# AnimatePortrait/AnimatePortrait

Hardware: AMD Instinct MI355X
Metric: generator frames/sec @256x256 bs=16 (higher is better)
Workload: dtype f32 (fp32 tensors; wide convs multiply fp32-class on the bf16 pipe: operands as bf16 head + tail, 3 products of 16-bit significands per multiply, ~2^-17 relative per product, fp32 accumulate); 1 GPU; Module2 generator resnet_9blocks_rcatland32_full_ifw fwd-only, ngf=64, bs=16/GPU, 256x256, fp32 (BASELINE configs[1]); global_batch=16, parallelism=dp1 (frame batches sharded, no collective), weights=random init N(0,0.02), seed 1234

## Files before the change

animateportrait_amd/csrc/conv_fwd.hip:

```cpp
#include "conv_plan.h"
#include "conv_direct.h"
#include "conv_tapgemm.h"
#include "conv_small.h"
#include "conv_head.h"
#include "conv_tsmall.h"

#include <cstdlib>
#include <cstring>

namespace apamd {

#ifdef APAMD_VARIANTS
const void* bf3_sb_kernel(size_t* lds_bytes);
#endif

static const void* direct_fn(int K, int cop) {
    if (K == 7 && cop == 1) return reinterpret_cast<const void*>(&conv_direct_f32<DirectCfg<7, 1>>);
    if (K == 7 && cop == 4) return reinterpret_cast<const void*>(&conv_direct_f32<DirectCfg<7, 4>>);
    return nullptr;
}
static size_t direct_lds_bytes(int K, int cop, int nbuf, int cin_pad) {
    if (cop == 1) return 4 * DirectCfg<7, 1>::lds_floats(nbuf, cin_pad);
    return 4 * DirectCfg<7, 4>::lds_floats(nbuf, cin_pad);
}

struct OutForm {
    const ap_out_view* view = nullptr;
    bool octet = false;
    bool bf16 = false;
};

struct FwdArgs {
    const float *packed, *bias;
    float *y, *stats;
    hipStream_t stream;
};

static int check_fwd_args(const ap_conv_desc* d, const Plan& pl, const OutForm& o, const FwdArgs& a) {
    if (o.bf16 && (!ob16_plan_ok(d, pl) || o.octet))
        return fail(AP_ERR_UNSUPPORTED, "conv2d_fwd_bf16out: only the plain-bf16 dense 3x3 stride-1 layers store bf16 (ap_conv2d_bf16out_ok)");
    if (!a.packed || !a.y) return fail(AP_ERR_INVALID, "null packed/y pointer");
    if (o.octet && !octet_plan_ok(d, pl))
        return fail(AP_ERR_UNSUPPORTED, "conv2d_fwd_octet: only single-launch split-bf16 layers of the run-time-tap / row kernel "
                                        "families with Cout %% 8 == 0 write the channel-octet layout (ap_conv2d_octet_ok)");
    if (o.view) {
        if (!pl.bf3 || pl.fused_phases || pl.launches.size() != 1)
            return fail(AP_ERR_UNSUPPORTED, "conv2d_fwd_view: only single-launch split-bf16 plans take an output window");
        if (o.view->OH < 1 || o.view->OW < 1 || o.view->OH > pl.Hout || o.view->OW > pl.Wout)
            return fail(AP_ERR_INVALID, "conv2d_fwd_view: window %dx%d outside the %dx%d output", o.view->OH, o.view->OW, pl.Hout, pl.Wout);
    }
    if (d->presplit && !pl.bf3) return fail(AP_ERR_INVALID, "desc.presplit set for a layer that does not take split sources");
    for (int s = 0; s < d->nsrc; ++s) {
        if (!d->src[s].data) return fail(AP_ERR_INVALID, "segment %d: null data", s);
        if ((d->src[s].mean == nullptr) != (d->src[s].rstd == nullptr))
            return fail(AP_ERR_INVALID, "segment %d: mean and rstd must be given together", s);
        if (d->src[s].act < 0 || d->src[s].act > 2) return fail(AP_ERR_INVALID, "segment %d: act %d", s, d->src[s].act);
    }
    return AP_OK;
}

static int launch_tsmall(const ap_conv_desc* d, const Plan& pl, const FwdArgs& a) {
    TSmallParams p;
    memset(&p, 0, sizeof(p));
    fill_seg(p.src, d->src[0], 0);
    p.N = d->N; p.C = pl.Cin; p.H = d->H; p.W = d->W; p.Cout = d->Cout;
    p.w = a.packed + pl.head_w_off; p.bias = a.bias; p.act = d->act; p.y = a.y;
    if (d->N > 65535 || (d->H + 7) / 8 > 65535) return fail(AP_ERR_UNSUPPORTED, "conv_tsmall: grid too large");
    const dim3 grid((d->W + 31) / 32, (d->H + 7) / 8, d->N);
    if (d->Cout == 1) hipLaunchKernelGGL((conv_tsmall_f32<1>), grid, dim3(256), 0, a.stream, p);
    else if (d->Cout == 2) hipLaunchKernelGGL((conv_tsmall_f32<2>), grid, dim3(256), 0, a.stream, p);
    else hipLaunchKernelGGL((conv_tsmall_f32<4>), grid, dim3(256), 0, a.stream, p);
    return check_launch("conv_tsmall_f32");
}

static int launch_head(const ap_conv_desc* d, const Plan& pl, const FwdArgs& a) {
    const int cus = num_cus();
    int rb = 3;
    long long best_cost = -1;
    for (int cand : {2, 3, 4, 5, 6, 10}) {
        const long long wgs = (long long)d->N * ((pl.Hout + cand - 1) / cand);
        const long long cost = ((wgs + cus - 1) / cus) * (cand + 3);
        if (best_cost < 0 || cost < best_cost) { rb = cand; best_cost = cost; }
    }
    HeadParams p;
    memset(&p, 0, sizeof(p));
    fill_seg(p.src, d->src[0], 0);
    p.N = d->N; p.C = pl.Cin; p.H = d->H; p.W = d->W; p.OH = pl.Hout; p.OW = pl.Wout;
    p.w = a.packed + pl.head_w_off; p.bias = a.bias; p.act = d->act; p.y = a.y;
    const dim3 hg(d->N, (pl.Hout + rb - 1) / rb);
    switch (rb) {
        case 2: hipLaunchKernelGGL(conv_head_fwd_kernel<2>, hg, dim3(1024), 0, a.stream, p); break;
        case 4: hipLaunchKernelGGL(conv_head_fwd_kernel<4>, hg, dim3(1024), 0, a.stream, p); break;
        case 5: hipLaunchKernelGGL(conv_head_fwd_kernel<5>, hg, dim3(1024), 0, a.stream, p); break;
        case 6: hipLaunchKernelGGL(conv_head_fwd_kernel<6>, hg, dim3(1024), 0, a.stream, p); break;
        case 10: hipLaunchKernelGGL(conv_head_fwd_kernel<10>, hg, dim3(1024), 0, a.stream, p); break;
        default: hipLaunchKernelGGL(conv_head_fwd_kernel<3>, hg, dim3(1024), 0, a.stream, p); break;
    }
    return check_launch("conv_head_fwd_kernel");
}

static int launch_small(const ap_conv_desc* d, const Plan& pl, const FwdArgs& a) {
    SmallKParams p;
    memset(&p, 0, sizeof(p));
    fill_seg(p.src, d->src[0], 0);
    p.N = d->N; p.H = d->H; p.W = d->W; p.Cin = pl.Cin; p.Cout = d->Cout; p.OH = pl.Hout; p.OW = pl.Wout;
    p.pad = d->pad; p.pad_mode = d->pad_mode;
    p.y = a.y; p.w = a.packed; p.bias = a.bias; p.act = d->act;
    p.stats = a.stats; p.stat_tiles = pl.stat_tiles;
    p.tiles_x = (pl.Wout + 31) / 32; p.tiles_y = (pl.Hout + 7) / 8;
    const dim3 grid((unsigned)((long long)d->N * p.tiles_y * p.tiles_x));
    if (d->stride == 1 && d->Cout == 8) hipLaunchKernelGGL((conv_small_f32<SmallCfg<1, 8>>), grid, dim3(256), 0, a.stream, p);
    else if (d->stride == 1) hipLaunchKernelGGL((conv_small_f32<SmallCfg<1, 16>>), grid, dim3(256), 0, a.stream, p);
    else if (d->Cout == 8) hipLaunchKernelGGL((conv_small_gather_f32<SmallCfg<2, 8>>), grid, dim3(256), 0, a.stream, p);
    else hipLaunchKernelGGL((conv_small_gather_f32<SmallCfg<2, 16>>), grid, dim3(256), 0, a.stream, p);
    return check_launch("conv_small_f32");
}

static bool tapgemm_serves(const ap_conv_desc* d, const Plan& pl, const FwdArgs& a) {
    return d->precision == AP_PRECISION_BF16X3 && d->Cout == 1 && d->KH == 7 && d->nsrc == 1 && d->src[0].C == TapGemmCfg::C &&
           d->pad_mode == AP_PAD_REFLECT && !a.stats && pl.cin_pad == TapGemmCfg::C;
}

static int launch_tapgemm(const ap_conv_desc* d, const Plan& pl, const FwdArgs& a) {
    const void* kfn = tapgemm_kernel();
    int rc = ensure_dyn_lds(kfn, 160 * 1024);
    if (rc) return rc;
    TapGemmParams p;
    memset(&p, 0, sizeof(p));
    fill_seg(p.seg, d->src[0], 0);
    p.N = d->N; p.H = d->H; p.W = d->W;
    p.y = a.y; p.wp = a.packed; p.bias = a.bias; p.act = d->act;
    p.tiles_x = (pl.Wout + TapGemmCfg::TW - 1) / TapGemmCfg::TW;
    const long long slots = 2LL * num_cus();
    long long best_cost = -1;
    for (int ty = 1; ty <= (pl.Hout + 7) / 8; ++ty) {
        const int th = (pl.Hout + ty - 1) / ty;
        const long long wgs = (long long)d->N * p.tiles_x * ((pl.Hout + th - 1) / th);
        const long long cost = ((wgs + slots - 1) / slots) * (th + 6);
        if (best_cost < 0 || cost < best_cost) { p.th = th; best_cost = cost; }
    }
    p.tiles_y = (pl.Hout + p.th - 1) / p.th;
    void* args[] = {&p};
    hipError_t e = hipLaunchKernel(kfn, dim3((unsigned)(d->N * p.tiles_y * p.tiles_x)), dim3(256), args, TapGemmCfg::lds_bytes(), a.stream);
    if (e != hipSuccess) return fail(AP_ERR_LAUNCH, "conv_tapgemm_bf16x3 launch: %s", hipGetErrorString(e));
    return AP_OK;
}

static int launch_direct(const ap_conv_desc* d, const Plan& pl, const FwdArgs& a) {
    if (tapgemm_serves(d, pl, a)) return launch_tapgemm(d, pl, a);
    const void* kfn = direct_fn(d->KH, pl.direct_cop);
    int rc = ensure_dyn_lds(kfn, 160 * 1024);
    if (rc) return rc;
    DirectKParams p;
    memset(&p, 0, sizeof(p));
    p.nseg = d->nsrc;
    for (int s = 0; s < d->nsrc; ++s) fill_seg(p.seg[s], d->src[s], pl.chunk_begin[s]);
    p.N = d->N; p.H = d->H; p.W = d->W; p.Cout = d->Cout; p.OH = pl.Hout; p.OW = pl.Wout;
    p.pad = d->pad; p.pad_mode = d->pad_mode;
    p.y = a.y; p.wp = a.packed; p.bias = a.bias; p.act = d->act;
    p.stats = a.stats; p.stat_tiles = pl.stat_tiles;
    p.nchunks = pl.nchunks; p.cin_pad = pl.cin_pad;
    p.tiles_x = (pl.Wout + 63) / 64; p.tiles_y = (pl.Hout + 15) / 16;
    const size_t lds = direct_lds_bytes(d->KH, pl.direct_cop, p.nchunks > 1 ? 2 : 1, p.cin_pad);
    void* args[] = {&p};
    hipError_t e = hipLaunchKernel(kfn, dim3((unsigned)(d->N * p.tiles_y * p.tiles_x)), dim3(256), args, lds, a.stream);
    if (e != hipSuccess) return fail(AP_ERR_LAUNCH, "conv_direct_f32 launch: %s", hipGetErrorString(e));
    return AP_OK;
}

static ConvKParams conv_params(const ap_conv_desc* d, const Plan& pl, const Launch& L, const FwdArgs& a, bool with_norm) {
    ConvKParams p;
    memset(&p, 0, sizeof(p));
    p.nseg = d->nsrc;
    for (int s = 0; s < d->nsrc; ++s) fill_seg(p.seg[s], d->src[s], pl.chunk_begin[s], with_norm);
    p.N = d->N; p.H = d->H; p.W = d->W; p.Cout = d->Cout;
    p.OH = L.OH; p.OW = L.OW; p.dy0 = L.dy0; p.dx0 = L.dx0;
    p.pad_mode = d->pad_mode; p.y = a.y;
    p.o_nstride = (long long)d->Cout * pl.Hout * pl.Wout; p.o_cstride = (long long)pl.Hout * pl.Wout; p.o_rstride = pl.Wout;
    p.osy = L.osy; p.osx = L.osx; p.oy_off = L.oy_off; p.ox_off = L.ox_off;
    p.wp = a.packed + L.wp_off; p.bias = a.bias; p.act = d->act;
    p.stats = a.stats; p.stat_tiles = pl.stat_tiles; p.stat_tile_off = L.stat_tile_off;
    p.ntaps = (int)L.taps.size(); p.nchunks = pl.nchunks;
    p.tiles_x = L.tiles_x; p.tiles_y = L.tiles_y; p.co_tiles = pl.co_tiles;
    p.cin_pad = pl.cin_pad;
// ... 214 lines not shown
```

animateportrait_amd/networks.py:

```python
import functools

import torch
import torch.nn as nn
from torch.optim import lr_scheduler

from . import ops
from .autograd import (conv_forward, materialize_forward, warp_forward, batch_split_forward,
                       generator_apply, discriminator_apply)
from .ops import (Feat, ConvSpec, ACT_NONE, ACT_RELU, ACT_LRELU, ACT_TANH, PAD_ZERO, PAD_REFLECT,
                  W_OIHW, W_IOHW)

GENERATOR_NAMES = ('resnet_9blocks_rcatland32_full_ifw', 'resnet_style2_9blocks')
_REFERENCE_ONLY_G = (
    'resnet_9blocks', 'resnet_9blocks_rcatland', 'resnet_9blocks_rcatland3',
    'resnet_9blocks_rcatland32', 'resnet_10blocks_rcatland32', 'resnet_9blocks_rcatland4',
    'resnet_9blocks_rcatland32_fw', 'resnet_9blocks_rcatland32_fw2', 'resnet_9blocks_rcatland32_ifw',
    'resnet_9blocks_rcatland32_ifw_single2', 'resnet_9blocks_rcatland32_full_ifw_colorcoded',
    'resnet_9blocks_rcatland32_full_ifw2', 'resnet_9blocks_rcatland32_full_ifw_single',
    'resnet_9blocks_rcatland32_full_ifw_single2', 'resnet_9blocks_rcatland32_full_ifw_single3', 'regressor',
    'combiner', 'resnet_9blocks_rcatland2', 'resnet_6blocks', 'unet_128', 'unet_256')


class ConvLayer(nn.Module):

    def __init__(self, cin_segments, cout, k, stride=1, pad=0, pad_mode=PAD_ZERO, transposed=False,
                 output_padding=0):
        super().__init__()
        cin = sum(cin_segments)
        shape = (cin, cout, k, k) if transposed else (cout, cin, k, k)
        self.weight = nn.Parameter(torch.empty(shape, dtype=torch.float32))
        self.bias = nn.Parameter(torch.zeros(cout, dtype=torch.float32))
        self.spec = ConvSpec(cin_segments, cout, k, stride, pad, pad_mode, transposed, output_padding,
                             W_IOHW if transposed else W_OIHW)
        self._slots = {}
        self._rows_spec = None
        self._s2d_spec = None

    def _packed(self, slot_id, spec, view):
        slot = ops.packed_slot(spec, self.weight, view, self._slots.get(slot_id))
        self._slots[slot_id] = slot
        return slot.buf

    def packed_dgrad(self, seg, spec, view):
        return self._packed(('dgrad', seg), spec, ops.WeightView(view))

    def packed(self):
        return self._packed('fwd', self.spec, ops.WeightView(self.weight.detach()))

    def run(self, srcs, norm_act=None, act=ACT_NONE, out_octet=False, out_bf16=False):
        if not isinstance(srcs, (list, tuple)):
            srcs = [srcs]
        spec, packed = self.spec, None
        if norm_act is None and ops.conv_d0_ok(spec, srcs, act):
            return ops.conv_d0(srcs[0], self.weight, self.bias.detach(), act)
        if ops.stem_rows_eligible(spec) and not srcs[0].is_split_only:
            spec, packed = self.rows_spec(), self.packed_rows()
            srcs = [ops.presplit_rows(srcs[0], self.spec.k, self.spec.pad, self.spec.pad_mode)]
        elif (srcs[0].s2d is not None or not srcs[0].is_split_only) and ops.s2d_eligible(spec, *srcs[0].data.shape[2:]):
            spec, packed = self.s2d_spec(), self.packed_s2d()
            if srcs[0].s2d is None:
                srcs[0].s2d = ops.presplit_s2d(srcs[0])
            srcs = [srcs[0].s2d]
        if packed is None:
            packed = self.packed()
        if norm_act is None:
            return ops.conv2d(spec, srcs, packed, self.bias.detach(), act=act, out_octet=out_octet)
        return ops.conv2d(spec, srcs, packed, None, want_stats=True, out_act=norm_act, out_octet=out_octet,
                          out_bf16=out_bf16 and spec is self.spec)

    def stages_split(self, shape):
        n, _, h, w = shape
        if ops.stem_rows_eligible(self.spec) or ops.s2d_eligible(self.spec, h, w):
            return False
        return ops.takes_split(self.spec, n, h, w)

    def s2d_spec(self):
        if self._s2d_spec is None:
            self._s2d_spec = ops.s2d_spec(self.spec)
        return self._s2d_spec

    def packed_s2d(self):
        return self._packed('s2d', self.s2d_spec(), ops.WeightView(self.weight.detach(), s2d_c=self.spec.cin_segments[0]))

    def rows_spec(self):
        if self._rows_spec is None:
            self._rows_spec = ops.stem_rows_spec(self.spec)
        return self._rows_spec

    def packed_rows(self):
        return self._packed('rows', self.rows_spec(), ops.WeightView(self.weight.detach(), rows_c=self.spec.cin_segments[0]))


def _seq(**children):
    return nn.ModuleDict({k.lstrip('_'): v for k, v in children.items()})


class ResnetBlock(nn.Module):

    def __init__(self, dim):
        super().__init__()
        self.conv_block = _seq(_1=ConvLayer([dim], dim, 3, 1, 1, PAD_REFLECT),
                               _5=ConvLayer([dim], dim, 3, 1, 1, PAD_REFLECT))

    def run(self, x, tape=None, consumer=None):
        c1, c5 = self.conv_block['1'], self.conv_block['5']
        dim = c1.spec.cout
        keep = consumer is not None and not consumer.stages_split(x.data.shape)
        y = conv_forward(tape, c1, x, norm_act=ACT_RELU, raw16=True, out_octet=tape is None and ops.trunk_octet_ok(dim))
        y = conv_forward(tape, c5, y, norm_act=ACT_NONE, raw16=True,
                         out_octet=tape is None and ops.trunk_octet_ok(dim, residual=x, keep_fp32=keep))
        return materialize_forward(tape, y, residual=x, consumer=consumer)


class ResnetBlock2(nn.Module):

    def __init__(self, segs, dim_out):
        super().__init__()
        self.conv_block = _seq(_1=ConvLayer(segs, dim_out, 3, 1, 1, PAD_REFLECT),
                               _5=ConvLayer([dim_out], dim_out, 3, 1, 1, PAD_REFLECT))
        self.shortcut = _seq(_0=ConvLayer(segs, dim_out, 3, 1, 1, PAD_ZERO))

    def run(self, srcs, tape=None, consumer=None):
        c1, c5, sc = self.conv_block['1'], self.conv_block['5'], self.shortcut['0']
        y = conv_forward(tape, c1, srcs, norm_act=ACT_RELU, raw16=True, out_octet=tape is None and ops.trunk_octet_ok(c1.spec.cout))
        y = conv_forward(tape, c5, y, norm_act=ACT_NONE, raw16=True)
        s = conv_forward(tape, sc, srcs, norm_act=ACT_NONE)
        return materialize_forward(tape, y, residual=s, consumer=consumer)


class ResnetConditionTriGenerator32_full_ifw(nn.Module):

    def __init__(self, input_nc, output_nc, ngf=64, norm='instance', use_dropout=False, n_blocks=9,
                 padding_type='reflect', div=3, disp=1):
        super().__init__()
        if norm != 'instance':
            raise NotImplementedError('normalization layer [%s] is not available on the HIP path' % norm)
        if use_dropout:
            raise NotImplementedError('dropout is not available on the HIP path (the model sets no_dropout)')
        if padding_type != 'reflect':
            raise NotImplementedError('padding [%s] is not implemented' % padding_type)
        assert n_blocks >= 0
        self.n_blocks, self.div, self.disp = n_blocks, div, disp
        self.input_nc, self.output_nc, self.ngf = input_nc, output_nc, ngf
        h = ngf // 2
        con_dim = 16
        dim = ngf * 4
        self.model_tri_merge = ConvLayer([ngf * 4, ngf * 4, ngf * 4], dim, 3, 1, 1)
        self.model_tri00 = _seq(_1=ConvLayer([input_nc], h, 7, 1, 3, PAD_REFLECT))
        self.model_tri01 = _seq(_0=ConvLayer([ngf], ngf * 2, 3, 2, 1))
        self.model_tri02 = _seq(_0=ConvLayer([ngf * 2], ngf * 4, 3, 2, 1))
        self.model_tri10 = _seq(_1=ConvLayer([input_nc], ngf, 7, 1, 3, PAD_REFLECT))
        self.model_tri11 = _seq(_0=ConvLayer([ngf], ngf, 3, 2, 1))
        self.model_tri12 = _seq(_0=ConvLayer([ngf * 2], ngf * 4, 3, 2, 1))
        self.model_tri20 = _seq(_1=ConvLayer([input_nc], ngf, 7, 1, 3, PAD_REFLECT))
        self.model_tri21 = _seq(_0=ConvLayer([ngf], ngf * 2, 3, 2, 1))
        self.model_tri22 = _seq(_0=ConvLayer([ngf * 2], ngf * 2, 3, 2, 1))
        blocks = {}
        for i in range(n_blocks):
            if (i + disp) % div == 0:
                blocks[str(i)] = ResnetBlock2([dim, con_dim, con_dim], dim)
            else:
                blocks[str(i)] = ResnetBlock(dim)
        self.model2 = nn.ModuleDict(blocks)
        self.model3 = _seq(_0=ConvLayer([ngf * 4], ngf * 2, 3, 2, 1, transposed=True, output_padding=1),
                           _3=ConvLayer([ngf * 2], ngf, 3, 2, 1, transposed=True, output_padding=1),
                           _7=ConvLayer([ngf], output_nc, 7, 1, 3, PAD_REFLECT))
        self.model_landmark_trans = _seq(_0=ConvLayer([1], 8, 3, 1, 1), _3=ConvLayer([8], con_dim, 3, 2, 1),
                                         _6=ConvLayer([con_dim], con_dim, 3, 2, 1))
        self.land1_cache_key = None
        self._land1_cache = None

    def is_block2(self, i):
        return (i + self.disp) % self.div == 0

    def double_feature_warping(self, x, motion, flow, ifmask, level, tape=None, consumer=None):
        return warp_forward(tape, x, motion, flow, ifmask, level, consumer=consumer)

    def forward(self, input, land1, land2, motion, flow, ifmask):
        if torch.is_grad_enabled() and (input.requires_grad or any(p.requires_grad for p in self.parameters())):
            return generator_apply(self, input, land1, land2, motion, flow, ifmask)
        return self.forward_inference(input, land1, land2, motion, flow, ifmask)

    def forward_inference(self, input, land1, land2, motion, flow, ifmask):
        return self._run(None, False, input, land1, land2, motion, flow, ifmask).data

    def _run(self, tape, input_needs_grad, input, land1, land2, motion, flow, ifmask):
        b = input.shape[0]
        inp = Feat(input.contiguous())
        if tape is not None and input_needs_grad:
            tape.track(inp)
        self._last_input_feat = inp if tape is not None else None
        motion, flow, ifmask = motion.contiguous(), flow.contiguous(), ifmask.contiguous()
        cf, dfw = conv_forward, self.double_feature_warping
        oct = tape is None

        def branch1():
            x = cf(tape, self.model_tri00['1'], inp, norm_act=ACT_RELU, out_octet=oct)
            x = dfw(x, motion, flow, ifmask, 0, tape, self.model_tri01['0'])
            x = cf(tape, self.model_tri01['0'], x, norm_act=ACT_RELU)
            return cf(tape, self.model_tri02['0'], x, norm_act=ACT_RELU)

        def branch2():
            x = cf(tape, self.model_tri10['1'], inp, norm_act=ACT_RELU)
            x = cf(tape, self.model_tri11['0'], x, norm_act=ACT_RELU, out_octet=oct)
            x = dfw(x, motion, flow, ifmask, 1, tape, self.model_tri12['0'])
            return cf(tape, self.model_tri12['0'], x, norm_act=ACT_RELU)

        def branch3():
            x = cf(tape, self.model_tri20['1'], inp, norm_act=ACT_RELU)
            x = cf(tape, self.model_tri21['0'], x, norm_act=ACT_RELU)
            x = cf(tape, self.model_tri22['0'], x, norm_act=ACT_RELU, out_octet=oct)
            return dfw(x, motion, flow, ifmask, 2, tape, self.model_tri_merge)

        def landmarks():
            lt = self.model_landmark_trans
            key = self.land1_cache_key
            if tape is None and key is not None:
                full = (key, tuple(land1.shape), tuple(ops.weight_key(lt[k].weight) for k in ('0', '3', '6')))
                if self._land1_cache is None or self._land1_cache[0] != full:
                    l = cf(None, lt['0'], Feat(land1.contiguous()), norm_act=ACT_RELU)
                    l = cf(None, lt['3'], l, norm_act=ACT_RELU)
                    l = cf(None, lt['6'], l, norm_act=ACT_NONE)
                    l.mean
                    self._land1_cache = (full, l)
                la = self._land1_cache[1]
                lb = cf(None, lt['0'], Feat(land2.contiguous()), norm_act=ACT_RELU)
                lb = cf(None, lt['3'], lb, norm_act=ACT_RELU)
                lb = cf(None, lt['6'], lb, norm_act=ACT_NONE)
                return la, lb
            lands = Feat(torch.cat([land1, land2], 0).contiguous())
            l = cf(tape, lt['0'], lands, norm_act=ACT_RELU)
            l = cf(tape, lt['3'], l, norm_act=ACT_RELU)
            l = cf(tape, lt['6'], l, norm_act=ACT_NONE)
            return batch_split_forward(tape, l, b)

        x1, x2, x3 = branch1(), branch2(), branch3()
        l1, l2 = landmarks()
        x = cf(tape, self.model_tri_merge, [x1, x2, x3])
        for i in range(self.n_blocks):
            blk = self.model2[str(i)]
            nxt = self.model3['0'] if i == self.n_blocks - 1 else None
            x = blk.run([x, l1, l2], tape, consumer=nxt) if self.is_block2(i) else blk.run(x, tape, consumer=nxt)
        x = cf(tape, self.model3['0'], x, norm_act=ACT_RELU)
        x = cf(tape, self.model3['3'], x, norm_act=ACT_RELU)
        return cf(tape, self.model3['7'], x, act=ACT_TANH)


class ResnetStyle2Generator(nn.Module):

    def __init__(self, input_nc, output_nc, ngf=64, norm='instance', use_dropout=False, n_blocks=6,
                 padding_type='reflect', extra_channel=3, model0_res=0):
        super().__init__()
        if norm != 'instance':
            raise NotImplementedError('normalization layer [%s] is not available on the HIP path' % norm)
        if use_dropout:
            raise NotImplementedError('dropout is not available on the HIP path')
        if padding_type != 'reflect':
            raise NotImplementedError('padding [%s] is not implemented' % padding_type)
        if model0_res != 0:
            raise NotImplementedError('model0_res != 0 is not used by any shipped configuration')
        assert n_blocks >= 0
        self.n_blocks = n_blocks
        dim = ngf * 4
        self.model0 = _seq(_1=ConvLayer([input_nc], ngf, 7, 1, 3, PAD_REFLECT),
                           _4=ConvLayer([ngf], ngf * 2, 3, 2, 1), _7=ConvLayer([ngf * 2], dim, 3, 2, 1))
        layers = {'0': ConvLayer([dim, extra_channel], dim, 3, 1, 1)}
        for i in range(n_blocks):
            layers[str(3 + i)] = ResnetBlock(dim)
        j = 3 + n_blocks
        layers[str(j)] = ConvLayer([dim], dim // 2, 3, 2, 1, transposed=True, output_padding=1)
        layers[str(j + 3)] = ConvLayer([dim // 2], dim // 4, 3, 2, 1, transposed=True, output_padding=1)
        layers[str(j + 7)] = ConvLayer([ngf], output_nc, 7, 1, 3, PAD_REFLECT)
        self.model = nn.ModuleDict(layers)

    def forward(self, input1, input2):
        with torch.no_grad():
            cf = conv_forward
            x = cf(None, self.model0['1'], Feat(input1.contiguous()), norm_act=ACT_RELU)
            x = cf(None, self.model0['4'], x, norm_act=ACT_RELU)
            x = cf(None, self.model0['7'], x, norm_act=ACT_RELU)
            x = cf(None, self.model['0'], [x, Feat(input2.contiguous())], norm_act=ACT_RELU)
            x = materialize_forward(None, x)
            j = 3 + self.n_blocks
            for i in range(self.n_blocks):
                x = self.model[str(3 + i)].run(x, None, consumer=self.model[str(j)] if i == self.n_blocks - 1 else None)
            x = cf(None, self.model[str(j)], x, norm_act=ACT_RELU)
            x = cf(None, self.model[str(j + 3)], x, norm_act=ACT_RELU)
            return cf(None, self.model[str(j + 7)], x, act=ACT_TANH).data


class P2CConv(ConvLayer):

    def __init__(self, cin, cout, k, stride=1, pad=0, pad_mode=PAD_ZERO, bias=False):
        super().__init__([cin], cout, k, stride, pad, pad_mode)
        self.spec.precision = ops.PRECISION_FP32
        nn.init.normal_(self.weight.data, 0.0, 0.02)
        if not bias:
            self.register_parameter('bias', None)

    def run(self, src, norm_act=None, act=ACT_NONE):
        if norm_act is None:
            return ops.conv2d(self.spec, [src], self.packed(), None if self.bias is None else self.bias.detach(), act=act)
        return ops.conv2d(self.spec, [src], self.packed(), None, want_stats=True, out_act=norm_act)


def _in_relu(t):
    return Feat(t[0], t[1], t[2], ACT_RELU)


class P2CConvBlock(nn.Module):

    def __init__(self, dim_in, dim_out):
        super().__init__()
        self.dim_in, self.dim_out = dim_in, dim_out
        self.ConvBlock1 = _seq(_3=P2CConv(dim_in, dim_out // 2, 3, 1, 1, PAD_REFLECT))
# ... 365 lines not shown
```

animateportrait_amd/ops.py:

```python
import collections
import ctypes
import os

import torch

from . import _capi as C
from ._capi import ACT_NONE, ACT_RELU, ACT_LRELU, ACT_TANH, PAD_ZERO, PAD_REFLECT, W_OIHW, W_IOHW

EPS = 1e-5

WEIGHTS_EPOCH = 0


def weight_key(w):
    owner = getattr(w, '_flat_owner', None)
    return (w._version, w.data_ptr(), WEIGHTS_EPOCH, owner.epoch if owner is not None else 0)

PRECISION_FP32, PRECISION_BF16X3, PRECISION_BF16 = 0, 1, 2
PRECISION_BY_NAME = {'fp32': PRECISION_FP32, 'bf16x3': PRECISION_BF16X3, 'bf16': PRECISION_BF16}
DEFAULT_PRECISION = PRECISION_BY_NAME.get(os.environ.get('APAMD_PRECISION', 'bf16x3'), PRECISION_BF16X3)


_LAST_STREAM = {}
_STREAM_FENCE = os.environ.get('APAMD_NO_STREAM_FENCE', '0') != '1'
# ... 442 lines not shown
    f.pending = None
    if want_xs and residual is None:
        f.xs = xs
        f.xs_heads_only = bool(flags & 1)
    return y, xs


def trunk_octet_ok(c, residual=None, keep_fp32=False):
    if (DEFAULT_PRECISION != PRECISION_BF16X3 or not RESIDUAL_AS_SPLIT or not OCTET_TRUNK or keep_fp32 or
            not wants_split(c) or c % 8):
        return False
    return residual is None or (residual.is_split_only and residual.xs is not None and not residual.xs_heads_only and residual.oct is None)


OCTET_TRUNK = os.environ.get('APAMD_NO_OCTET_TRUNK', '0') != '1'


def wants_split(c):
    return DEFAULT_PRECISION != PRECISION_FP32 and c >= 48 and c % 16 == 0


def takes_split(spec, n, h, w):
    if spec.precision == PRECISION_FP32:
        return False
    d = spec.desc(n, h, w)
    return bool(C.check(C.lib().ap_conv2d_wants_presplit(ctypes.byref(d)), 'wants_presplit'))


def conv2d(spec, srcs, packed, bias=None, act=ACT_NONE, want_stats=False, out_act=ACT_NONE, out_octet=False, out_bf16=False):
    x0 = srcs[0].data
    n, _, h, w = x0.shape
    for f, c in zip(srcs, spec.cin_segments):
        if not f.is_split_only:
            _require_device(f.data, 'conv input', allow_bf16=True)
        if f.data.shape[1] != c or f.data.shape[0] != n or f.data.shape[2:] != x0.shape[2:]:
            raise ValueError('conv2d: source of shape %s does not match segment C=%d' % (tuple(f.data.shape), c))
    d = spec.desc(n, h, w, None, act)
    lib = C.lib()
    if spec.precision != PRECISION_FP32 and C.check(lib.ap_conv2d_wants_presplit(ctypes.byref(d)), 'wants_presplit'):
        if spec.precision == PRECISION_BF16X3 and DEFAULT_PRECISION == PRECISION_BF16:
            raise RuntimeError('a split-bf16 (bf16x3) layer cannot run while the package mode is plain bf16: split copies '
                               'are then written without their tail planes')
        spec.presplit_desc(n, h, w, srcs, d=d)
    else:
        if any(f.is_split_only for f in srcs):
            raise RuntimeError('conv2d: a source exists only as its split-bf16 copy but this layer reads fp32')
        if any(f.data.dtype != torch.float32 for f in srcs):
            raise RuntimeError('conv2d: a source holds bf16 values but this layer reads fp32')
        spec.fill_sources(d, srcs)
    ho, wo = ctypes.c_int32(), ctypes.c_int32()
    C.check(lib.ap_conv2d_out_size(ctypes.byref(d), ctypes.byref(ho), ctypes.byref(wo)), 'conv2d_out_size')
    out_octet = bool(out_octet) and d.presplit == 1 and lib.ap_conv2d_octet_ok(ctypes.byref(d)) == 1
    out_bf16 = bool(out_bf16) and not out_octet and d.presplit == 1 and lib.ap_conv2d_bf16out_ok(ctypes.byref(d)) == 1
    if out_octet:
        y = torch.empty((n, spec.cout // 8, ho.value * wo.value, 8), dtype=torch.float32, device=x0.device)
    else:
        y = torch.empty((n, spec.cout, ho.value, wo.value), dtype=torch.bfloat16 if out_bf16 else torch.float32, device=x0.device)
    partial = None
    if want_stats:
        tiles = C.check(lib.ap_conv2d_stat_tiles(ctypes.byref(d)), 'conv2d_stat_tiles')
        partial = torch.empty((n * spec.cout, tiles, 2), dtype=torch.float32, device=x0.device)
    if PROFILER is not None:
        buf = ctypes.create_string_buffer(96)
        C.check(lib.ap_conv2d_kernel_name(ctypes.byref(d), buf, 96), 'conv2d_kernel_name')
        e0, e1 = torch.cuda.Event(enable_timing=True), torch.cuda.Event(enable_timing=True)
        e0.record()
    fwd = lib.ap_conv2d_fwd_octet if out_octet else (lib.ap_conv2d_fwd_bf16out if out_bf16 else lib.ap_conv2d_fwd)
    C.check(fwd(ctypes.byref(d), _ptr(packed), _ptr(bias), _ptr(y), _ptr(partial), _stream()), 'conv2d_fwd')
    if PROFILER is not None:
        e1.record()
        px = h * w if spec.transposed else ho.value * wo.value
        macs = getattr(spec, 'alg_macs', None) or sum(spec.cin_segments) * spec.k ** 2
        PROFILER.records.append((buf.value.decode(), 2.0 * n * px * spec.cout * macs, e0, e1))
    if out_octet:
        res = Feat(_stand_in((n, spec.cout, ho.value, wo.value), x0.device),
                   act=out_act if want_stats else ACT_NONE, pending=(partial, tiles) if want_stats else None)
        res.oct = y
        return res
    if not want_stats:
        return Feat(y)
    return Feat(y, act=out_act, pending=(partial, tiles))


RESIDUAL_AS_SPLIT = True
K7_WGRAD = os.environ.get('APAMD_NO_K7_WGRAD', '0') != '1'
D0_MFMA = K7_WGRAD and os.environ.get('APAMD_NO_D0_MFMA', '0') != '1'


def _conv2d_view(spec, srcs, packed, out, view):
    x0 = srcs[0].data
    n, _, h, w = x0.shape
    d = spec.presplit_desc(n, h, w, srcs)
    fn = C.lib().ap_conv2d_fwd_view_bf16out if out.dtype == torch.bfloat16 else C.lib().ap_conv2d_fwd_view
    C.check(fn(ctypes.byref(d), ctypes.byref(view), _ptr(packed), None, _ptr(out), _stream()), 'conv2d_fwd_view')


def dgrad_strip_eligible(spec, g):
    if (spec.precision == PRECISION_FP32 or spec.k != 3 or spec.stride != 1 or spec.pad != 2 or spec.transposed or
            len(spec.cin_segments) != 1 or g.virtual):
        return False
    n, c, h, w = g.shape
    if (w + 2) % 32 != 2 or w < 32 or h < 4 or c % 8:
        return False
    d = spec.desc(n, h, w, None, ACT_NONE)
    return bool(C.check(C.lib().ap_conv2d_wants_presplit(ctypes.byref(d)), 'wants_presplit'))


def conv2d_dgrad_strip(spec, g, packed, packed_t, strip=None, out_bf16=False):
    n, c, h, w = g.data.shape
    hp, wp = h + 2, w + 2
    out_bf16 = bool(out_bf16) and C.lib().ap_conv2d_bf16out_ok(ctypes.byref(spec.presplit_desc(n, h, w))) == 1
    out = torch.empty((n, spec.cout, hp, wp), dtype=torch.bfloat16 if out_bf16 else torch.float32, device=g.data.device)
    if strip is None and g.is_split_only:
        raise RuntimeError('conv2d_dgrad_strip: the gradient exists only as its split copy and no column strip was prepared '
                           '(ap_instnorm_bwd_split writes it when the backward plan asks for one)')
    t = strip if strip is not None else Feat(g.data[:, :, :, w - 2:].transpose(2, 3).contiguous())
    _conv2d_view(spec, [t], packed_t, out, C.ApOutView(spec.cout * hp * wp, hp * wp, 1, wp, w - 2, 0, 4, hp))
    _conv2d_view(spec, [g], packed, out, C.ApOutView(spec.cout * hp * wp, hp * wp, wp, 1, 0, 0, hp, w))
    return out


def materialize(f, residual=None, emit_xs=None, keep_fp32=True):
    if not f.virtual:
        raise ValueError('materialize: feature is already plain')
    n, c, h, w = f.data.shape
    if emit_xs is None:
        emit_xs = wants_split(c)
    if c % 8 == 0:
        split_only = (bool(emit_xs) and not keep_fp32 and RESIDUAL_AS_SPLIT and
                      DEFAULT_PRECISION == PRECISION_BF16X3)
        if residual is not None and residual.is_split_only and not split_only and residual.xs_heads_only:
            raise RuntimeError('materialize: the residual exists only as a head-only split copy')
        y, xs = _norm_apply_split(f, residual, want_y=not split_only, want_xs=bool(emit_xs))
        out = Feat.split_only((n, c, h, w), xs) if split_only else Feat(y)
        out.xs = xs
        out.xs_heads_only = xs is not None and DEFAULT_PRECISION == PRECISION_BF16
        return out
    x = f.data
    out = torch.empty_like(x)
    res = rm = rr = None
    if residual is not None:
        if residual.act != ACT_NONE and residual.virtual:
            raise ValueError('materialize: a normalised residual cannot carry an activation')
        res, rm, rr = residual.data, residual.mean, residual.rstd
        if res.shape != x.shape:
            raise ValueError('materialize: residual shape mismatch')
    C.check(C.lib().ap_instnorm_apply(_ptr(x), _ptr(f.mean), _ptr(f.rstd), f.act, _ptr(res), _ptr(rm), _ptr(rr),
                                      _ptr(out), n * c, h * w, _stream()), 'instnorm_apply')
    return Feat(out)


def warp_concat(f, motion, flow, ifmask, level, emit_xs=False, keep_fp32=True, s2d=False):
    x = f.data
    n, c, h, w = x.shape
    if f.oct is not None:
        x = f.oct
    for t, name in ((x, 'x'), (motion, 'motion'), (flow, 'flow'), (ifmask, 'ifmask')):
        _require_device(t, name)
    s = motion.shape[1]
    if motion.shape != (n, s, s, 2) or flow.shape != (n, 2, s, s) or ifmask.shape != (n, 1, s, s):
        raise ValueError('warp_concat: motion/flow/ifmask shapes %s %s %s' % (motion.shape, flow.shape, ifmask.shape))
    if h != s >> level or w != s >> level:
        raise ValueError('warp_concat: level %d expects %d px features, got %dx%d' % (level, s >> level, h, w))
    emit_xs = bool(emit_xs) and c % 8 == 0
    s2d = bool(s2d) and emit_xs and h % 2 == 0 and w % 2 == 0
    out = xs = None
# ... 502 lines not shown
```

include/animateportrait_amd.h:

```cpp
#ifndef ANIMATEPORTRAIT_AMD_H
#define ANIMATEPORTRAIT_AMD_H

#include <stdint.h>

#ifdef __cplusplus
extern "C" {
#endif

typedef void* ap_stream_t;

enum { AP_OK = 0, AP_ERR_INVALID = -1, AP_ERR_UNSUPPORTED = -2, AP_ERR_LAUNCH = -3 };
enum { AP_ACT_NONE = 0, AP_ACT_RELU = 1, AP_ACT_LRELU = 2 , AP_ACT_TANH = 3 };
enum { AP_PAD_ZERO = 0, AP_PAD_REFLECT = 1 };
enum { AP_W_OIHW = 0 , AP_W_IOHW = 1  };
enum { AP_PRECISION_FP32 = 0, AP_PRECISION_BF16X3 = 1, AP_PRECISION_BF16 = 2 };

typedef struct ap_src {
    const float* data;
    const float* mean;
    const float* rstd;
    int32_t C;
    int32_t act;
} ap_src;

typedef struct ap_conv_desc {
    int32_t N, H, W;
    int32_t Cout;
    int32_t KH, KW;
    int32_t stride;
    int32_t pad;
    int32_t pad_mode;
    int32_t transposed;
    int32_t output_padding;
    int32_t w_layout;
    int32_t w_flip;
    int32_t act;
    int32_t nsrc;
    int32_t precision;
    int32_t presplit;
    int32_t s2d_k;
    ap_src src[3];
} ap_conv_desc;

#define AP_ABI_VERSION 16
int32_t ap_abi_version(void);
const char* ap_version(void);
const char* ap_last_error(void);

int ap_conv2d_out_size(const ap_conv_desc* d, int32_t* Hout, int32_t* Wout);
int64_t ap_conv2d_packed_floats(const ap_conv_desc* d);
int32_t ap_conv2d_stat_tiles(const ap_conv_desc* d);
int ap_conv2d_pack_weights(const ap_conv_desc* d, const float* weight, float* packed, ap_stream_t stream);

typedef struct ap_weight_view {
    const float* w;
    int64_t s_co, s_ci, s_ky, s_kx;
    int32_t s2d_c, rows_c, ksrc, reserved;
} ap_weight_view;
int32_t ap_conv2d_pack_entry_bytes(void);
int32_t ap_conv2d_pack_entries(const ap_conv_desc* d, const ap_weight_view* v, float* packed, void* entries, int32_t max_entries);
int ap_conv2d_pack_run(const void* entries_dev, int32_t count, ap_stream_t stream);
int ap_conv2d_fwd(const ap_conv_desc* d, const float* packed, const float* bias, float* y,
                  float* stat_partials, ap_stream_t stream);
typedef struct ap_out_view {
    int64_t nstride, cstride;
    int32_t rstride, xstride, y_off, x_off, OH, OW;
} ap_out_view;
int ap_conv2d_fwd_view(const ap_conv_desc* d, const ap_out_view* view, const float* packed, const float* bias, float* y,
                       ap_stream_t stream);
int32_t ap_conv2d_octet_ok(const ap_conv_desc* d);
int ap_conv2d_fwd_octet(const ap_conv_desc* d, const float* packed, const float* bias, float* y, float* stat_partials,
                        ap_stream_t stream);
int32_t ap_conv2d_bf16out_ok(const ap_conv_desc* d);
int ap_conv2d_fwd_bf16out(const ap_conv_desc* d, const float* packed, const float* bias, void* y_bf16, float* stat_partials,
                          ap_stream_t stream);
int ap_conv2d_fwd_view_bf16out(const ap_conv_desc* d, const ap_out_view* view, const float* packed, const float* bias, void* y_bf16,
                               ap_stream_t stream);

int32_t ap_conv2d_wants_presplit(const ap_conv_desc* d);
int64_t ap_split_prepass_bytes(int32_t N, int32_t C, int32_t H, int32_t W);
int ap_split_prepass(const ap_src* src, int32_t N, int32_t H, int32_t W, void* out, ap_stream_t stream);
int ap_split_prepass_rows(const ap_src* src, int32_t N, int32_t H, int32_t W, int32_t K, int32_t pad, int32_t pad_mode,
                          void* out, ap_stream_t stream);
int ap_split_prepass_s2d(const ap_src* src, int32_t N, int32_t H, int32_t W, void* out, ap_stream_t stream);
int ap_norm_apply_split(const ap_src* src, const float* stat_partials, int32_t tiles, float eps, float* mean_out,
                        float* rstd_out, const ap_src* residual, int32_t N, int32_t H, int32_t W, float* y, void* xs,
                        ap_stream_t stream);
int ap_norm_apply_split_ex(const ap_src* src, const float* stat_partials, int32_t tiles, float eps, float* mean_out,
                           float* rstd_out, const ap_src* residual, int32_t N, int32_t H, int32_t W, float* y, void* xs,
                           int32_t flags, ap_stream_t stream);

int ap_conv2d_kernel_name(const ap_conv_desc* d, char* buf, int32_t buflen);

int ap_instnorm_finalize(const float* stat_partials, const float* y, int32_t NC, int32_t tiles, int32_t count,
                         float eps, float* mean, float* rstd, ap_stream_t stream);
int ap_instnorm_finalize_octet(const float* stat_partials, const float* y, int32_t N, int32_t C, int32_t tiles, int32_t count,
                               float eps, float* mean, float* rstd, ap_stream_t stream);
int ap_instnorm_apply(const float* x, const float* mean, const float* rstd, int32_t act,
                      const float* res, const float* res_mean, const float* res_rstd,
                      float* out, int32_t NC, int32_t HW, ap_stream_t stream);

int ap_warp_concat_fwd(const float* x, const float* x_mean, const float* x_rstd, int32_t x_act,
                       const float* motion, const float* flow, const float* ifmask,
                       float* out, int32_t N, int32_t C, int32_t H, int32_t W, int32_t S,
                       float flow_scale, ap_stream_t stream);
int ap_motion_grid(const float* pts, const float* val, const int32_t* tri, int32_t N, int32_t P, int32_t T, int32_t S,
// ... 129 lines not shown
```

Baseline: 2426 frames/s.

## Fuse landmark encoder layers 0 and 1 by recomputing layer-0 output on the fly

Replaces the stored 1->8 stride-1 landmark conv (with its full 8-channel activation write and reread) by a statistics-only pass that produces instance-norm sums, followed by a fused kernel. The fused kernel recomputes the 1->8 conv per tile in shared memory, applies norm and ReLU, and runs the 8->16 stride-2 conv with its stats epilogue. This removes the largest intermediate memory traffic of the landmark branch. In exchange it computes layer 0 twice and adds a halo of redundant work per tile.

```diff
diff --git a/animateportrait_amd/csrc/conv_fwd.hip b/animateportrait_amd/csrc/conv_fwd.hip
--- a/animateportrait_amd/csrc/conv_fwd.hip
+++ b/animateportrait_amd/csrc/conv_fwd.hip
@@ -2,6 +2,7 @@
 #include "conv_direct.h"
 #include "conv_tapgemm.h"
 #include "conv_small.h"
+#include "conv_land.h"
 #include "conv_head.h"
 #include "conv_tsmall.h"
 
@@ -36,10 +37,23 @@
     hipStream_t stream;
 };
 
+static bool land0_stats_serves(const ap_conv_desc* d, const Plan& pl, const OutForm& o, const FwdArgs& a) {
+    return pl.small && pl.Cin == 1 && d->Cout == kLandC0 && d->stride == 1 && d->pad == 1 && d->pad_mode == AP_PAD_ZERO &&
+           !d->src[0].mean && !d->src[0].rstd && d->src[0].act == AP_ACT_NONE && !a.bias && a.stats && !o.view && !o.octet && !o.bf16;
+}
+static bool land01_serves(const ap_conv_desc* d, const Plan& pl, const OutForm& o, const FwdArgs& a) {
+    return pl.small && pl.Cin == kLandC0 && d->Cout == kLandC1 && d->stride == 2 && d->pad == 1 && d->pad_mode == AP_PAD_ZERO &&
+           d->src[0].mean && d->src[0].rstd && d->src[0].act == (AP_SRC_LAND0 | AP_ACT_RELU) && d->act == AP_ACT_NONE && !a.bias &&
+           a.stats && !o.view && !o.octet && !o.bf16;
+}
+
 static int check_fwd_args(const ap_conv_desc* d, const Plan& pl, const OutForm& o, const FwdArgs& a) {
     if (o.bf16 && (!ob16_plan_ok(d, pl) || o.octet))
         return fail(AP_ERR_UNSUPPORTED, "conv2d_fwd_bf16out: only the plain-bf16 dense 3x3 stride-1 layers store bf16 (ap_conv2d_bf16out_ok)");
-    if (!a.packed || !a.y) return fail(AP_ERR_INVALID, "null packed/y pointer");
+    if (!a.packed || (!a.y && !land0_stats_serves(d, pl, o, a))) return fail(AP_ERR_INVALID, "null packed/y pointer");
+    if ((d->src[0].act & AP_SRC_LAND0) && !land01_serves(d, pl, o, a))
+        return fail(AP_ERR_UNSUPPORTED, "AP_SRC_LAND0: only the 8 -> 16 stride-2 zero-padded 3x3 layer behind a 1 -> 8 one recomputes its "
+                                        "source (statistics given, ReLU, raw output with a statistics epilogue, no bias)");
     if (o.octet && !octet_plan_ok(d, pl))
         return fail(AP_ERR_UNSUPPORTED, "conv2d_fwd_octet: only single-launch split-bf16 layers of the run-time-tap / row kernel "
                                         "families with Cout %% 8 == 0 write the channel-octet layout (ap_conv2d_octet_ok)");
@@ -54,7 +68,8 @@
         if (!d->src[s].data) return fail(AP_ERR_INVALID, "segment %d: null data", s);
         if ((d->src[s].mean == nullptr) != (d->src[s].rstd == nullptr))
             return fail(AP_ERR_INVALID, "segment %d: mean and rstd must be given together", s);
-        if (d->src[s].act < 0 || d->src[s].act > 2) return fail(AP_ERR_INVALID, "segment %d: act %d", s, d->src[s].act);
+        const int sact = s == 0 ? d->src[s].act & ~AP_SRC_LAND0 : d->src[s].act;
+        if (sact < 0 || sact > 2) return fail(AP_ERR_INVALID, "segment %d: act %d", s, d->src[s].act);
     }
     return AP_OK;
 }
@@ -99,7 +114,23 @@
     return check_launch("conv_head_fwd_kernel");
 }
 
+static int launch_land(const ap_conv_desc* d, const Plan& pl, const FwdArgs& a) {
+    LandParams p;
+    memset(&p, 0, sizeof(p));
+    p.x = d->src[0].data; p.N = d->N; p.H = d->H; p.W = d->W; p.OH = pl.Hout; p.OW = pl.Wout;
+    p.stats = a.stats; p.stat_tiles = pl.stat_tiles;
+    p.tiles_x = (pl.Wout + 31) / 32; p.tiles_y = (pl.Hout + 7) / 8;
+    if (!a.y) {
+        p.w0 = a.packed;
+        return launch_land0_stats(p, a.stream);
+    }
+    p.w1 = a.packed; p.w0 = a.packed + kLandC1 * kLandC0 * 9;
+    p.mean = d->src[0].mean; p.rstd = d->src[0].rstd; p.y = a.y;
+    return launch_land01_fused(p, a.stream);
+}
+
 static int launch_small(const ap_conv_desc* d, const Plan& pl, const FwdArgs& a) {
+    if (!a.y || (d->src[0].act & AP_SRC_LAND0)) return launch_land(d, pl, a);
     SmallKParams p;
     memset(&p, 0, sizeof(p));
     fill_seg(p.src, d->src[0], 0);
diff --git a/animateportrait_amd/csrc/conv_land.h b/animateportrait_amd/csrc/conv_land.h
--- /dev/null
+++ b/animateportrait_amd/csrc/conv_land.h
@@ -0,0 +1,206 @@
+#pragma once
+#include "conv_small.h"
+
+namespace apamd {
+
+constexpr int kLandC0 = 8, kLandC1 = 16;
+constexpr int kLandStatK = 8;
+
+struct LandParams {
+    const float* x;
+    const float* w0;
+    const float* w1;
+    const float* mean;
+    const float* rstd;
+    float* y;
+    float* stats;
+    int N, H, W, OH, OW, stat_tiles, tiles_x, tiles_y;
+};
+
+int launch_land0_stats(const LandParams& p, hipStream_t stream);
+int launch_land01_fused(const LandParams& p, hipStream_t stream);
+
+__device__ __forceinline__ void land0_pixel(const float (&x)[9], const float (&w)[kLandC0 * 9], float (&v)[kLandC0]) {
+#pragma unroll
+    for (int c = 0; c < kLandC0; ++c) {
+        float acc = 0.f;
+#pragma unroll
+        for (int t = 0; t < 9; ++t) acc += x[t] * w[c * 9 + t];
+        v[c] = acc;
+    }
+}
+
+__device__ __forceinline__ int clampi(int i, int n) { return i < 0 ? 0 : (i >= n ? n - 1 : i); }
+
+template <int K>
+__global__ __launch_bounds__(256) void land0_stats_kernel(const LandParams p) {
+    __shared__ double red[4][2 * kLandC0];
+    const int tid = threadIdx.x, lx = tid & 31, ly = tid >> 5;
+    const int groups = (p.stat_tiles + K - 1) / K;
+    const int n = blockIdx.x / groups, g = blockIdx.x - n * groups;
+    const int H = p.H, W = p.W;
+    float w[kLandC0 * 9];
+#pragma unroll
+    for (int i = 0; i < kLandC0 * 9; ++i) w[i] = p.w0[i];
+    const float* plane = p.x + (long long)n * H * W;
+    double s[kLandC0], q[kLandC0];
+#pragma unroll
+    for (int c = 0; c < kLandC0; ++c) s[c] = q[c] = 0.0;
+#pragma unroll
+    for (int k = 0; k < K; ++k) {
+        int t = g * K + k;
+        const bool have = t < p.stat_tiles;
+        t = have ? t : p.stat_tiles - 1;
+        const int tiy = t / p.tiles_x, tix = t - tiy * p.tiles_x;
+        const int oy = tiy * 8 + ly, ox = tix * 32 + lx;
+        const bool live = have && oy < H && ox < W;
+        float raw[9];
+#pragma unroll
+        for (int j = 0; j < 9; ++j) raw[j] = plane[clampi(oy + j / 3 - 1, H) * W + clampi(ox + j % 3 - 1, W)];
+        float x[9];
+#pragma unroll
+        for (int j = 0; j < 9; ++j) {
+            const int iy = oy + j / 3 - 1, ix = ox + j % 3 - 1;
+            x[j] = (iy >= 0 && iy < H && ix >= 0 && ix < W) ? raw[j] : 0.f;
+        }
+        float v[kLandC0];
+        land0_pixel(x, w, v);
+#pragma unroll
+        for (int c = 0; c < kLandC0; ++c) {
+            const double d = live ? (double)v[c] : 0.0;
+            s[c] += d;
+            q[c] += d * d;
+        }
+    }
+#pragma unroll
+    for (int c = 0; c < kLandC0; ++c) {
+#pragma unroll
+        for (int sh = 1; sh < 64; sh <<= 1) {
+            s[c] += __shfl_xor(s[c], sh, 64);
+            q[c] += __shfl_xor(q[c], sh, 64);
+        }
+    }
+    if ((tid & 63) == 0) {
+#pragma unroll
+        for (int c = 0; c < kLandC0; ++c) { red[tid >> 6][c] = s[c]; red[tid >> 6][kLandC0 + c] = q[c]; }
+    }
+    __syncthreads();
+    if (tid < kLandC0) {
+        const double S = red[0][tid] + red[1][tid] + red[2][tid] + red[3][tid];
+        const double Q = red[0][kLandC0 + tid] + red[1][kLandC0 + tid] + red[2][kLandC0 + tid] + red[3][kLandC0 + tid];
+        const int left = p.stat_tiles - g * K, cnt = left < K ? left : K;
+        float2* d = reinterpret_cast<float2*>(p.stats) + ((long long)(n * kLandC0 + tid) * p.stat_tiles + g * K) * 2;
+        const float sh = (float)S, qh = (float)Q;
+        d[0] = make_float2(sh, qh);
+        d[1] = make_float2((float)(S - (double)sh), (float)(Q - (double)qh));
+        for (int j = 2; j < 2 * cnt; ++j) d[j] = make_float2(0.f, 0.f);
+    }
+}
+
+template <class C>
+__global__ __launch_bounds__(256) void land01_fused_kernel(const LandParams p) {
+    constexpr int TH = C::TH, TW = C::TW, C0 = kLandC0, C1 = C::COUT;
+    static_assert(C::S == 2 && C1 == kLandC1 && TH == 8 && TW == 32, "tile of the 8 -> 16 stride-2 layer");
+    constexpr int LH = 2 * TH + 1, LW = 2 * TW + 1;
+    constexpr int XH = LH + 2, XW = LW + 2, XP = XW + 1;
+    constexpr int LP = (LW + 1) / 2;
+    constexpr int NX = (XH * XW + 255) / 256;
+    __shared__ __attribute__((aligned(16))) float wl[C0 * 9 * C1];
+    __shared__ float xin[XH * XP];
+    __shared__ float xl[C0 * LH * 2 * LP];
+    __shared__ float red[8][C1][2];
+    const int tid = threadIdx.x, lx = tid & 31, ly = tid >> 5;
+    int b = (int)xcd_logical_block(gridDim.x, blockIdx.x);
+    const int tix = b % p.tiles_x; b /= p.tiles_x;
+    const int tiy = b % p.tiles_y;
+    const int n = b / p.tiles_y;
+    const int H = p.H, W = p.W;
+    const int gy0 = tiy * TH * 2 - 2, gx0 = tix * TW * 2 - 2;
+    const float* plane = p.x + (long long)n * H * W;
+    float raw[NX];
+#pragma unroll
+    for (int i = 0; i < NX; ++i) {
+        const int e = tid + i * 256, ty = e / XW, tx = e - ty * XW;
+        raw[i] = plane[clampi(gy0 + ty, H) * W + clampi(gx0 + tx, W)];
+    }
+    float w[C0 * 9], m[C0], r[C0];
+#pragma unroll
+    for (int i = 0; i < C0 * 9; ++i) w[i] = p.w0[i];
+#pragma unroll
+    for (int c = 0; c < C0; ++c) { m[c] = p.mean[n * C0 + c]; r[c] = p.rstd[n * C0 + c]; }
+    for (int i = tid; i < C0 * 9 * C1; i += 256) {
+        const int co = i % C1, t = (i / C1) % 9, ci = i / (9 * C1);
+        wl[i] = p.w1[(co * C0 + ci) * 9 + t];
+    }
+#pragma unroll
+    for (int i = 0; i < NX; ++i) {
+        const int e = tid + i * 256, ty = e / XW, tx = e - ty * XW;
+        const int iy = gy0 + ty, ix = gx0 + tx;
+        if (e < XH * XW) xin[ty * XP + tx] = (iy >= 0 && iy < H && ix >= 0 && ix < W) ? raw[i] : 0.f;
+    }
+    __syncthreads();
+    for (int e = tid; e < LH * LW; e += 256) {
+        const int wy = e / LW, wx = e - wy * LW;
+        float x[9];
+#pragma unroll
+        for (int t = 0; t < 9; ++t) x[t] = xin[(wy + t / 3) * XP + wx + t % 3];
+        float v[C0];
+        land0_pixel(x, w, v);
+        const int gy = gy0 + 1 + wy, gx = gx0 + 1 + wx;
+        const bool inside = gy >= 0 && gy < H && gx >= 0 && gx < W;
+        float* dst = xl + (wy * 2 + (wx & 1)) * LP + (wx >> 1);
+#pragma unroll
+        for (int c = 0; c < C0; ++c) {
+            const float u = fmaxf((v[c] - m[c]) * r[c], 0.f);
+            dst[c * LH * 2 * LP] = inside ? u : 0.f;
+        }
+    }
+    __syncthreads();
+    const int oy = tiy * TH + ly, ox = tix * TW + lx;
+    const bool live = oy < p.OH && ox < p.OW;
+    float acc[C1];
+#pragma unroll
+    for (int co = 0; co < C1; ++co) acc[co] = 0.f;
+    for (int c = 0; c < C0; ++c) {
+        const float* xp = xl + (c * LH + 2 * ly) * 2 * LP + lx;
+        float x[9];
+#pragma unroll
+        for (int t = 0; t < 9; ++t) x[t] = xp[((t / 3) * 2 + ((t % 3) & 1)) * LP + ((t % 3) >> 1)];
+#pragma unroll
+        for (int t = 0; t < 9; ++t) {
+            const float4* wv = reinterpret_cast<const float4*>(wl + (c * 9 + t) * C1);
+#pragma unroll
+            for (int q = 0; q < C1 / 4; ++q) {
+                const float4 w4 = wv[q];
+                acc[q * 4 + 0] += x[t] * w4.x;
+                acc[q * 4 + 1] += x[t] * w4.y;
+                acc[q * 4 + 2] += x[t] * w4.z;
+                acc[q * 4 + 3] += x[t] * w4.w;
+            }
+        }
+    }
+    float sv[C1], qv[C1];
+#pragma unroll
+    for (int co = 0; co < C1; ++co) {
+        const float v = acc[co];
+        if (live) p.y[((long long)n * C1 + co) * p.OH * p.OW + oy * p.OW + ox] = v;
+        sv[co] = live ? v : 0.f;
+        qv[co] = live ? v * v : 0.f;
+    }
+    int co_s, co_q;
+    const float s = halfwave_sums<C1>(sv, lx, co_s);
+    const float q = halfwave_sums<C1>(qv, lx, co_q);
+    constexpr int GROUP = 32 / C1;
+    if ((lx & (GROUP - 1)) == 0) { red[ly][co_s][0] = s; red[ly][co_q][1] = q; }
+    __syncthreads();
+    if (tid < C1) {
+        float s2 = 0.f, q2 = 0.f;
+#pragma unroll
+        for (int r8 = 0; r8 < 8; ++r8) { s2 += red[r8][tid][0]; q2 += red[r8][tid][1]; }
+        float* d = p.stats + (((long long)n * C1 + tid) * p.stat_tiles + tiy * p.tiles_x + tix) * 2;
+        d[0] = s2;
+        d[1] = q2;
+    }
+}
+
+}
diff --git a/animateportrait_amd/csrc/conv_land_inst.hip b/animateportrait_amd/csrc/conv_land_inst.hip
--- /dev/null
+++ b/animateportrait_amd/csrc/conv_land_inst.hip
@@ -0,0 +1,20 @@
+#include "conv_land.h"
+
+namespace apamd {
+
+int launch_land0_stats(const LandParams& p, hipStream_t stream) {
+    const long long groups = (p.stat_tiles + kLandStatK - 1) / kLandStatK;
+    if (p.N * groups > 0x7fffffffLL || (long long)p.N * kLandC0 * p.H * p.W > 0x7fffffffLL)
+        return fail(AP_ERR_UNSUPPORTED, "land0_stats: grid too large");
+    hipLaunchKernelGGL(land0_stats_kernel<kLandStatK>, dim3((unsigned)(p.N * groups)), dim3(256), 0, stream, p);
+    return check_launch("land0_stats_kernel");
+}
+
+int launch_land01_fused(const LandParams& p, hipStream_t stream) {
+    const long long nblk = (long long)p.N * p.tiles_y * p.tiles_x;
+    if (nblk > 0x7fffffffLL || (long long)p.H * p.W > 0x7fffffffLL) return fail(AP_ERR_UNSUPPORTED, "land01_fused: grid too large");
+    hipLaunchKernelGGL((land01_fused_kernel<SmallCfg<2, 16>>), dim3((unsigned)nblk), dim3(256), 0, stream, p);
+    return check_launch("land01_fused_kernel");
+}
+
+}
diff --git a/animateportrait_amd/networks.py b/animateportrait_amd/networks.py
--- a/animateportrait_amd/networks.py
+++ b/animateportrait_amd/networks.py
@@ -89,6 +89,22 @@
 
     def packed_rows(self):
         return self._packed('rows', self.rows_spec(), ops.WeightView(self.weight.detach(), rows_c=self.spec.cin_segments[0]))
+
+
+def _land_packed01(l0, l1):
+    key = (ops.weight_key(l0.weight), ops.weight_key(l1.weight))
+    c = l1._slots.get('land01')
+    if c is None or c[0] != key:
+        c = (key, torch.cat([l1.weight.detach().reshape(-1), l0.weight.detach().reshape(-1)]))
+        l1._slots['land01'] = c
+    return c[1]
+
+
+def landmark_encode01(lt, x, tape=None):
+    if tape is None and ops.land_fused_ok(lt['0'].spec, lt['3'].spec, x):
+        return ops.land_encode01(lt['0'].spec, lt['3'].spec, lt['0'].packed(), _land_packed01(lt['0'], lt['3']), x)
+    l = conv_forward(tape, lt['0'], Feat(x), norm_act=ACT_RELU)
+    return conv_forward(tape, lt['3'], l, norm_act=ACT_RELU)
 
 
 def _seq(**children):
@@ -215,22 +231,19 @@
         def landmarks():
             lt = self.model_landmark_trans
             key = self.land1_cache_key
+
+            def encode01(x):
+                return landmark_encode01(lt, x, tape)
             if tape is None and key is not None:
                 full = (key, tuple(land1.shape), tuple(ops.weight_key(lt[k].weight) for k in ('0', '3', '6')))
                 if self._land1_cache is None or self._land1_cache[0] != full:
-                    l = cf(None, lt['0'], Feat(land1.contiguous()), norm_act=ACT_RELU)
-                    l = cf(None, lt['3'], l, norm_act=ACT_RELU)
-                    l = cf(None, lt['6'], l, norm_act=ACT_NONE)
+                    l = cf(None, lt['6'], encode01(land1.contiguous()), norm_act=ACT_NONE)
                     l.mean
                     self._land1_cache = (full, l)
                 la = self._land1_cache[1]
-                lb = cf(None, lt['0'], Feat(land2.contiguous()), norm_act=ACT_RELU)
-                lb = cf(None, lt['3'], lb, norm_act=ACT_RELU)
-                lb = cf(None, lt['6'], lb, norm_act=ACT_NONE)
+                lb = cf(None, lt['6'], encode01(land2.contiguous()), norm_act=ACT_NONE)
                 return la, lb
-            lands = Feat(torch.cat([land1, land2], 0).contiguous())
-            l = cf(tape, lt['0'], lands, norm_act=ACT_RELU)
-            l = cf(tape, lt['3'], l, norm_act=ACT_RELU)
+            l = encode01(torch.cat([land1, land2], 0).contiguous())
             l = cf(tape, lt['6'], l, norm_act=ACT_NONE)
             return batch_split_forward(tape, l, b)
 
diff --git a/animateportrait_amd/ops.py b/animateportrait_amd/ops.py
--- a/animateportrait_amd/ops.py
+++ b/animateportrait_amd/ops.py
@@ -548,6 +548,55 @@
     return Feat(y, act=out_act, pending=(partial, tiles))
 
 
+SRC_LAND0 = 0x200
+
+
+def land_stored():
+    return int(os.environ.get('APAMD_LAND_STORED', '0') or 0) != 0
+
+
+def land_fused_ok(spec0, spec1, x):
+    def is3(s, cin, cout, stride):
+        return (s.cin_segments == (cin,) and s.cout == cout and s.k == 3 and s.stride == stride and s.pad == 1 and
+                s.pad_mode == PAD_ZERO and not s.transposed and s.w_layout == W_OIHW and not s.w_flip and s.kh is None)
+    n, c, h, w = x.shape
+    return (not land_stored() and int(os.environ.get('APAMD_NO_SMALL', '0') or 0) == 0 and is3(spec0, 1, 8, 1) and
+            is3(spec1, 8, 16, 2) and c == 1 and x.dtype == torch.float32 and n * 16 * h * w < 2 ** 31)
+
+
+def land0_stats(spec0, w0, x):
+    _require_device(x, 'landmark map')
+    n, _, h, w = x.shape
+    lib = C.lib()
+    d = spec0.desc(n, h, w, [Feat(x)])
+    tiles = 2 * C.check(lib.ap_conv2d_stat_tiles(ctypes.byref(d)), 'conv2d_stat_tiles')
+    partial = torch.empty((n * spec0.cout, tiles, 2), dtype=torch.float32, device=x.device)
+    C.check(lib.ap_conv2d_fwd(ctypes.byref(d), _ptr(w0), None, None, _ptr(partial), _stream()), 'conv2d_fwd (statistics only)')
+    mean = torch.empty(n * spec0.cout, dtype=torch.float32, device=x.device)
+    rstd = torch.empty_like(mean)
+    C.check(lib.ap_instnorm_finalize(_ptr(partial), None, n * spec0.cout, tiles, h * w, EPS, _ptr(mean), _ptr(rstd), _stream()),
+            'instnorm_finalize')
+    return mean, rstd
+
+
+def land_encode01(spec0, spec1, w0, w10, x, out_act=ACT_RELU):
+    n, _, h, w = x.shape
+    mean, rstd = land0_stats(spec0, w0, x)
+    lib = C.lib()
+    d = spec1.desc(n, h, w)
+    d.src[0].data, d.src[0].C = x.data_ptr(), spec0.cout
+    d.src[0].mean, d.src[0].rstd, d.src[0].act = mean.data_ptr(), rstd.data_ptr(), SRC_LAND0 | ACT_RELU
+    ho, wo = ctypes.c_int32(), ctypes.c_int32()
+    C.check(lib.ap_conv2d_out_size(ctypes.byref(d), ctypes.byref(ho), ctypes.byref(wo)), 'conv2d_out_size')
+    tiles = C.check(lib.ap_conv2d_stat_tiles(ctypes.byref(d)), 'conv2d_stat_tiles')
+    y = torch.empty((n, spec1.cout, ho.value, wo.value), dtype=torch.float32, device=x.device)
+    partial = torch.empty((n * spec1.cout, tiles, 2), dtype=torch.float32, device=x.device)
+    C.check(lib.ap_conv2d_fwd(ctypes.byref(d), _ptr(w10), None, _ptr(y), _ptr(partial), _stream()), 'conv2d_fwd (landmark layers 0 + 1)')
+    if PROFILER is not None:
+        PROFILER.note('land01_fused')
+    return Feat(y, act=out_act, pending=(partial, tiles))
+
+
 RESIDUAL_AS_SPLIT = True
 K7_WGRAD = os.environ.get('APAMD_NO_K7_WGRAD', '0') != '1'
 D0_MFMA = K7_WGRAD and os.environ.get('APAMD_NO_D0_MFMA', '0') != '1'
diff --git a/include/animateportrait_amd.h b/include/animateportrait_amd.h
--- a/include/animateportrait_amd.h
+++ b/include/animateportrait_amd.h
@@ -22,6 +22,7 @@
     int32_t C;
     int32_t act;
 } ap_src;
+enum { AP_SRC_LAND0 = 0x200 };
 
 typedef struct ap_conv_desc {
     int32_t N, H, W;
```

Result: no change. 2424 frames/s (-0.1%).
